# musaru/Fall_Multimodal

Measured on AMD Instinct MI355X. Metric: clips/sec (fwd+bwd) 3-stream Fall3, B=256, 1/2/4/8 GPUs; top-1 acc parity, higher is better.
Workload: dtype bf16x3; 1 GPU; fall3_3stream_coco_mmpose_V18_S6_B256_per_gpu; global_batch=256, seq_len=30, parallelism=dp1, joints=18, imu_axes=6, classes=11, hip_graph=False, ranks=1

## Files before the change

fall_multimodal_amd/_lib.py:

```python
from __future__ import annotations

import ctypes
import os

import torch

HERE = os.path.dirname(os.path.abspath(__file__))
LIB_PATH = os.environ.get("F3_LIB") or os.path.join(HERE, "libfall3.so")

EXPORTS = (
    "f3_net_create", "f3_net_destroy", "f3_net_num_entries", "f3_net_entry", "f3_net_param_count",
    "f3_net_buffer_count", "f3_net_counter_count", "f3_net_workspace_bytes", "f3_net_forward",
    "f3_net_loss", "f3_net_backward", "f3_rmsprop_step", "f3_conv_forward", "f3_status_string",
    "f3_net_debug_tensor", "f3_conv_backward_data", "f3_conv_backward_weight", "f3_conv_wgrad_packed", "f3_split_x3cat",
    "f3_conv_forward_x3cat", "f3_conv_backward_data_x3cat", "f3_conv_backward_weight_x3cat", "f3_conv_step_x3cat", "f3_graph_mix_forward",
    "f3_graph_mix_backward", "f3_graph_mix_forward_ex", "f3_graph_mix_backward_ex", "f3_gcn_dgrad_mix_x3",
    "f3_gcn_fwd_mix_x3",
    "f3_net_backward_phase",
    "f3_net_grad_split", "f3_net_wait_phase1", "f3_net_backward_rmsprop", "f3_net_fused_rmsprop", "f3_net_precision", "f3_net_status",
    "f3_targcn_create", "f3_targcn_destroy", "f3_targcn_num_entries", "f3_targcn_entry", "f3_targcn_param_count",
    "f3_targcn_buffer_count", "f3_targcn_workspace_bytes", "f3_targcn_forward", "f3_targcn_backward", "f3_targcn_stage_times", "f3_targcn_status", "f3_net_sensor_times", "f3_soft_ce",
    "f3_sktr_create", "f3_sktr_destroy", "f3_sktr_num_entries", "f3_sktr_entry", "f3_sktr_param_count",
    "f3_sktr_buffer_count", "f3_sktr_counter_count", "f3_sktr_workspace_bytes", "f3_sktr_forward", "f3_sktr_backward",
    "f3_musa_create", "f3_musa_destroy", "f3_musa_num_entries", "f3_musa_entry", "f3_musa_param_count",
    "f3_musa_buffer_count", "f3_musa_counter_count", "f3_musa_workspace_bytes", "f3_musa_forward", "f3_musa_backward",
    "f3_musa_guards",
    "f3_dwconv_t_forward", "f3_pointwise_conv", "f3_rgb_scratch_floats", "f3_rgb_forward", "f3_rgb_backward",
    "f3_optim_scalars_bytes", "f3_optim_step", "f3_optim_step_ranges", "f3_net_backward_optim", "f3_net_entry_nograd",
    "f3_metrics_bytes", "f3_metrics_reset", "f3_metrics_update", "f3_segment_norms_scratch_bytes", "f3_segment_norms",
    "f3_soft_ce_ex", "f3_net_loss_ex", "f3_grad_accumulate",
    "f3_optim_hyper_bytes", "f3_optim_hyper_set", "f3_optim_step_hyper",
)

F3_OK, F3_EINVAL, F3_EBATCH, F3_EHIP, F3_ESTATE, F3_EDEVICE = 0, 1001, 1002, 1003, 1004, 1005
ENTRY_PARAM, ENTRY_BUFFER, ENTRY_COUNTER = 0, 1, 2
OPT_RMSPROP, OPT_SGD, OPT_ADAM, OPT_ADAMW = 0, 1, 2, 3
OPT_MAX_SKIP = 4
METRICS_MAXK, METRICS_MAXC = 8, 64


# ... 69 lines not shown
        "f3_metrics_update": (I, [P, P, P, P, P, I, I, ctypes.POINTER(I), I, P]),
        "f3_segment_norms_scratch_bytes": (I64, [I64, I]),
        "f3_segment_norms": (I, [P, P, P, I, P, P, I64, ctypes.c_double, P]),
        "f3_soft_ce_ex": (I, [P, P, P, I, I, F, P, P, P]),
        "f3_net_loss_ex": (I, [P, I, P, P, F, P, P, P]),
        "f3_grad_accumulate": (I, [P, P, I64, P, P]),
        "f3_conv_forward": (I, [P, P, P, P, P, I, I, I, I, I, I, I, I, I, P]),
        "f3_status_string": (ctypes.c_char_p, [I]),
        "f3_net_debug_tensor": (P, [P, I, P, I, I, ctypes.c_char_p]),
        "f3_conv_backward_data": (I, [P, P, P, P, I, I, I, I, I, I, I, I, I, P]),
        "f3_conv_backward_weight": (I, [P, P, P, P, I, I, I, I, I, I, I, I, I, P]),
        "f3_conv_wgrad_packed": (I, [P, P, P, ctypes.c_longlong, I, I, I, I, I, I, I, I, P]),
        "f3_split_x3cat": (I, [P, P, ctypes.c_int64, I, P]),
        "f3_conv_forward_x3cat": (I, [P, P, P, P, P, I, I, I, I, I, I, I, I, P]),
        "f3_conv_backward_data_x3cat": (I, [P, P, P, P, I, I, I, I, I, I, I, I, P]),
        "f3_conv_backward_weight_x3cat": (I, [P, P, P, P, I, I, I, I, I, I, I, I, P]),
        "f3_conv_step_x3cat": (I, [I, P, P, P, P, P, P, P, P, P, P, F, P, P, I, I, I, I, I, P]),
        "f3_graph_mix_forward": (I, [P, P, P, I, I, I, I, P]),
        "f3_graph_mix_backward": (I, [P, P, P, P, P, I, I, I, I, P]),
        "f3_graph_mix_forward_ex": (I, [P, P, P, I, I, I, I, I, P]),
        "f3_graph_mix_backward_ex": (I, [P, P, P, P, P, I, I, I, I, I, P]),
        "f3_gcn_dgrad_mix_x3": (I, [P, P, P, P, P, P, P, I, I, I, I, I, I, I, P]),
        "f3_gcn_fwd_mix_x3": (I, [P, P, P, P, P, P, P, P, P, I, I, I, I, I, P]),
        "f3_targcn_create": (I, [ctypes.POINTER(F3TargcnConfig), ctypes.POINTER(P)]),
        "f3_targcn_destroy": (None, [P]),
        "f3_targcn_num_entries": (I, [P]),
        "f3_targcn_entry": (I, [P, I, ctypes.POINTER(ctypes.c_char_p), ctypes.POINTER(I), ctypes.POINTER(I),
                                ctypes.POINTER(I64), ctypes.POINTER(I64)]),
        "f3_targcn_param_count": (I64, [P]),
        "f3_targcn_buffer_count": (I64, [P]),
        "f3_targcn_workspace_bytes": (I64, [P, I]),
        "f3_targcn_stage_times": (I, [P, I, P]),
        "f3_targcn_status": (I, [P, I]),
        "f3_net_sensor_times": (I, [P, I, P]),
        "f3_targcn_forward": (I, [P, I, P, P, P, P, P, P]),
        "f3_targcn_backward": (I, [P, I, P, P, P, P, P, P]),
        "f3_soft_ce": (I, [P, P, I, I, P, P, P]),
        "f3_sktr_create": (I, [ctypes.POINTER(F3SktrConfig), ctypes.POINTER(P)]),
        "f3_sktr_destroy": (None, [P]),
        "f3_sktr_num_entries": (I, [P]),
        "f3_sktr_entry": (I, [P, I, ctypes.POINTER(ctypes.c_char_p), ctypes.POINTER(I), ctypes.POINTER(I),
                              ctypes.POINTER(I64), ctypes.POINTER(I64)]),
        "f3_sktr_param_count": (I64, [P]),
        "f3_sktr_buffer_count": (I64, [P]),
        "f3_sktr_counter_count": (I64, [P]),
        "f3_sktr_workspace_bytes": (I64, [P, I]),
# ... 49 lines not shown
```

fall_multimodal_amd/csrc/kernel_entries.cpp:

```cpp
#include <hip/hip_runtime.h>

#include <cstring>

#include "common.h"
#include "kernels.h"
#include "layers.h"
#include "host_args.h"
#include "fall3.h"

using namespace f3;

extern "C" {

static const unsigned short* test_zero_page() {
  static void* z = nullptr;
  if (!z && hipMalloc(&z, 4096) == hipSuccess) (void)hipMemset(z, 0, 4096);
  return (const unsigned short*)z;
}
static float* test_scratch(size_t n) {
  static float* p = nullptr;
  static size_t cap = 0;
  if (n > cap) {
    if (p) (void)hipFree(p);
    p = nullptr;
// ... 326 lines not shown
}

int f3_gcn_fwd_mix_x3(const float* A_eff, const float* x, const float* w, void* wpack, const float* bias_v, void* z3,
                      float* g, double* st_sum, double* st_sq, int frames, int K, int V, int Cin, int C,
                      void* stream) {
  hipStream_t s = (hipStream_t)stream;
  if (!A_eff || !x || !wpack || !bias_v || !z3 || !g || !st_sum || !st_sq || frames < 0) return F3_EINVAL;
  if (!f3_gcn_fwd_mix_ok(K, V, Cin, C)) return F3_EINVAL;
  if (w) {
    PrepTable t;
    t.n = 0;
    add_job(t, PREP_PACK_CONV, C * K * Cin * x3mul(x3code()), static_cast<float*>(wpack), w, nullptr, nullptr, C,
            K * Cin, 1, x3code());
    F3_TRY(f3_prep(t, s));
  }
  GcnFwdMixArgs a;
  std::memset(&a, 0, sizeof(a));
  a.frames = frames; a.K = K; a.V = V; a.Cin = Cin; a.C = C; a.A = A_eff; a.x = x;
  a.z3 = static_cast<unsigned short*>(z3); a.w = static_cast<const unsigned short*>(wpack); a.bias = bias_v; a.g = g;
  a.st_sum = st_sum; a.st_sq = st_sq; a.zero = test_zero_page();
  return f3_gcn_fwd_mix(&a, s);
}

}
```

fall_multimodal_amd/csrc/layers.h:

```cpp
#pragma once
#include "common.h"

namespace f3 {

enum : int { PREP_MUL = 0, PREP_PACK_CONV, PREP_PACK_CONV_T, PREP_PACK_GCN, PREP_PACK_GCN_T, PREP_GCN_BIAS, PREP_COPY,
              PREP_UNPACK_CONV };

struct PrepJob {
  int type, n;
  float* dst;
  const float* s0;
  const float* s1;
  const float* s2;
  int d0, d1, d2;
  int bf16;
};

struct DataBnArgs {
  int N, T, V, C, motion;
  const float* skel;
  float* out;
  int act16;
  BnRef bn;
  double* st_sum;
// ... 96 lines not shown
  unsigned short* outb;
  const float* dout;
  const float* dout_nc;
  float* P1;
  float* P2;
  float* Q2;
  double* bnr_bsum;
  double* bnr_bsq;
  const double* bn2_bsum;
  const double* bn2_bsq;
  const float* e;
  float* dh;
  float* dres;
  unsigned short* dhb;
  unsigned short* dresb;
  int x3;
  float* dgamma2;
  float* dbeta2;
  float* part;
  float* dgammar;
  float* dbetar;
  float* dbpart;
  int no_colsum;
};

struct BnBwdArgs {
  int N, TV, C, V, chunks;
  int act16;
  BnRef bn;
  const double* bsum;
  const double* bsq;
  float* dgamma;
  float* dbeta;
  const float* dv;
  const float* g;
  float* dg;
  float* G;
  float* Gpart;
  unsigned short* dgb;
  int no_colsum;
  int x3;
};

struct BnReluArgs {
  int M, C;
  int g16;
// ... 68 lines not shown
int f3_databn_bwd(const f3::DataBnArgs* a, hipStream_t s);
int f3_mix_fwd(const f3::MixArgs* a, hipStream_t s);
int f3_mix_bwd(const f3::MixArgs* a, hipStream_t s);
int f3_mix_bwd_parts(const f3::MixArgs* a);
bool f3_gcn_dgrad_mix_ok(int K, int V, int Cin, int C);
int f3_gcn_dgrad_mix(const f3::GcnDgradMixArgs* a, hipStream_t s);
int f3_gcn_dgrad_mix_parts(const f3::GcnDgradMixArgs* a);
bool f3_gcn_fwd_mix_ok(int K, int V, int Cin, int C);
int f3_gcn_fwd_mix(const f3::GcnFwdMixArgs* a, hipStream_t s);
bool f3_mix_lds_ok(int K, int V, int Cin);
bool f3_mix_x3_ok(int K, int V, int Cin);
int f3_split_x3(const float* x, unsigned short* out, long long rows, int C, hipStream_t s);
int f3_gcn_bias_bwd(const f3::GcnBiasBwdArgs* a, hipStream_t s);
bool f3_gcn0_ok(int K, int V, int Ci, int C);
int f3_gcn0_fwd(const f3::Gcn0Args* a, hipStream_t s);
int f3_gcn0_bwd(const f3::Gcn0Args* a, hipStream_t s);
int f3_gcn0_bwd_parts(const f3::Gcn0Args* a);
int f3_databn_bwd2(const f3::DataBnArgs* a, hipStream_t s);
int f3_block_out(f3::BlockArgs a, hipStream_t s);
int f3_block_bwd_reduce(f3::BlockArgs a, hipStream_t s);
int f3_block_bwd_apply(f3::BlockArgs a, hipStream_t s);
int f3_bn_bwd_apply(f3::BnBwdArgs a, hipStream_t s);
int f3_bn_bwd_parts(int N, int TV, int V);
int f3_block_chunks(int TV);
int f3_bnrelu_bf16(const f3::BnReluArgs* a, hipStream_t s);
constexpr int kColsumJobs = 10;
struct ColsumJob {
  const float* part;
  float* out;
  long long ld;
  int rows, cols;
};
int f3_colsum_multi(const ColsumJob* jobs, int n, hipStream_t s);
int f3_colsum(const float* part, int rows, int cols, float* out, hipStream_t s);
int f3_colsum_ld(const float* part, int rows, long long ld, int cols, float* out, hipStream_t s);
int f3_ca_fwd(const f3::CaArgs* a, hipStream_t s);
int f3_ca_bwd(const f3::CaArgs* a, hipStream_t s);
int f3_ca_bwd_weights(const f3::CaArgs* a, hipStream_t s, ColsumJob* defer = nullptr, int* ndefer = nullptr);
bool f3_ca_x_ok(int N, int C, int TV);
int f3_bn_running(const f3::BnRunTable& t, hipStream_t s);
```

fall_multimodal_amd/csrc/layers.hip:

```cpp
#include "common.h"
#include "layers.h"

#include <algorithm>
#include <cstring>
#include <type_traits>

namespace f3 {

typedef __bf16 bf16x4 __attribute__((ext_vector_type(4)));
typedef __bf16 bf16x8 __attribute__((ext_vector_type(8)));

F3_DEV void prep_x3n(const PrepJob& j, int e) {
  const bool gcn = j.type == PREP_PACK_GCN || j.type == PREP_PACK_GCN_T;
  const bool tr = j.type == PREP_PACK_CONV_T || j.type == PREP_PACK_GCN_T;
  const int J = j.d0, I = j.d1, KT = gcn ? 1 : j.d2;
  const int inner = gcn ? (tr ? J : j.d2 * I) : (tr ? J : I);
  const int row = e / (KT * inner), r = e - row * KT * inner, dt = r / inner, c = r - dt * inner;
  float val;
  if (gcn) {
    const int kc = tr ? row : c, cc = tr ? c : row, k = kc / I, ci = kc - k * I;
    val = j.s0[((size_t)k * J + cc) * I + ci];
  } else {
    val = tr ? j.s0[((size_t)c * I + row) * KT + dt] : j.s0[((size_t)row * I + c) * KT + dt];
  }
// ... 953 lines not shown
}

F3_DEV void chunk_rows(int TV, int chunks, int& r0, int& r1) {
  const int n = blockIdx.y, ch = blockIdx.x;
  const int per = (TV + chunks - 1) / chunks;
  r0 = n * TV + ch * per;
  r1 = min(n * TV + TV, r0 + per);
}

F3_DEV f32x4 quad_reduce(f32x4 v, float* lds, int C4) {
  const int tid = threadIdx.x;
  __syncthreads();
  reinterpret_cast<f32x4*>(lds)[tid] = v;
  __syncthreads();
  f32x4 r = {0.f, 0.f, 0.f, 0.f};
  if (tid < C4) {
    for (int i = tid; i < 256; i += C4) r += reinterpret_cast<f32x4*>(lds)[i];
  }
  return r;
}

constexpr int kRowU = 4;

template <bool A16, int RES>
__global__ __launch_bounds__(256) void block_out_kernel(BlockArgs a) {
  __shared__ __attribute__((aligned(16))) float lds[1024];
  const int C = a.C, C4 = C / 4, RP = 256 / C4, tid = threadIdx.x;
  int r0, r1;
  chunk_rows(a.TV, a.chunks, r0, r1);
  const int n = blockIdx.y, cq = tid % C4, c0 = cq * 4;
  const int mb0 = r0 + tid / C4;
  f32x4 h[kRowU], res[kRowU];
  size_t off[kRowU];
#define F3_BO_LOADS(MB)                                                  \
  _Pragma("unroll") for (int u = 0; u < kRowU; ++u) {                    \
    off[u] = (size_t)min((MB) + u * RP, r1 - 1) * C + c0;                \
    h[u] = ld_act4<A16>(a.h, off[u]);                                    \
    if (RES == RES_CONV) res[u] = ld_act4<A16>(a.r, off[u]);             \
    else if (RES == RES_ID) res[u] = ld_act4<A16>(a.x, off[u]);          \
    else res[u] = f32x4{0.f, 0.f, 0.f, 0.f};                             \
  }
  F3_BO_LOADS(mb0)
  float sc2[4], sh2[4], scr[4], shr[4], mu[4], rs[4];
  bn_coeff4(a.bn2, c0, sc2, sh2, mu, rs);
  if (RES == RES_CONV) bn_coeff4(a.bnr, c0, scr, shr, mu, rs);
  const f32x4 av = *reinterpret_cast<const f32x4*>(a.att + (size_t)n * C + c0);
  f32x4 pool = {0.f, 0.f, 0.f, 0.f};
  for (int mb = mb0; mb < r1; mb += kRowU * RP) {
    if (mb != mb0) F3_BO_LOADS(mb)
#pragma unroll
    for (int u = 0; u < kRowU; ++u) {
      f32x4 o;
#pragma unroll
      for (int e = 0; e < 4; ++e) {
        float rv = res[u][e];
        if (RES == RES_CONV) rv = rv * scr[e] + shr[e];
        o[e] = fmaxf((h[u][e] * sc2[e] + sh2[e]) * av[e] + rv, 0.f);
      }
      st_act4<A16>(a.out, off[u], o);
      if (a.outb) {
        bf16x4 ob, lb;
#pragma unroll
        for (int e = 0; e < 4; ++e) {
          ob[e] = (__bf16)o[e];
          lb[e] = (__bf16)(o[e] - (float)ob[e]);
        }
        if (a.x3) {
          __bf16* row = reinterpret_cast<__bf16*>(a.outb) + 2 * (off[u] - c0) + c0;
          *reinterpret_cast<bf16x4*>(row) = ob;
          *reinterpret_cast<bf16x4*>(row + C) = lb;
        } else {
          *reinterpret_cast<bf16x4*>(reinterpret_cast<__bf16*>(a.outb) + off[u]) = ob;
        }
      }
      if (mb + u * RP < r1) pool += o;
    }
  }
#undef F3_BO_LOADS
  if (a.pool) {
    f32x4 r = quad_reduce(pool, lds, C4);
    if (tid < C4) {
      if (a.part) {
        *reinterpret_cast<f32x4*>(a.part + ((size_t)blockIdx.x * a.N + n) * C + tid * 4) = r * a.inv_tv;
      } else {
#pragma unroll
        for (int e = 0; e < 4; ++e) atomic_add_f(a.pool + (size_t)n * C + tid * 4 + e, r[e] * a.inv_tv);
      }
    }
  }
}

template <bool A16, int RES, bool DNC>
__global__ __launch_bounds__(256) void block_bwd_reduce_kernel(BlockArgs a) {
  __shared__ __attribute__((aligned(16))) float lds[1024];
  const int C = a.C, C4 = C / 4, RP = 256 / C4, tid = threadIdx.x;
  int r0, r1;
  chunk_rows(a.TV, a.chunks, r0, r1);
  const int n = blockIdx.y, cq = tid % C4, c0 = cq * 4;
  const int mb0 = r0 + tid / C4;
  f32x4 o[kRowU], d[kRowU], h[kRowU], rr[kRowU];
#define F3_BR_LOADS(MB)                                                          \
  _Pragma("unroll") for (int u = 0; u < kRowU; ++u) {                            \
    const size_t off = (size_t)min((MB) + u * RP, r1 - 1) * C + c0;              \
    o[u] = ld_act4<A16>(a.out, off);                                             \
    if (!DNC) d[u] = *reinterpret_cast<const f32x4*>(a.dout + off);              \
    h[u] = ld_act4<A16>(a.h, off);                                               \
    if (RES == RES_CONV) rr[u] = ld_act4<A16>(a.r, off);                         \
  }
  F3_BR_LOADS(mb0)
  float mu2[4], rs2[4], mur[4], rsr[4], sc[4], sh[4];
  bn_coeff4(a.bn2, c0, sc, sh, mu2, rs2);
  if (RES == RES_CONV) bn_coeff4(a.bnr, c0, sc, sh, mur, rsr);
  f32x4 p1 = {0, 0, 0, 0}, p2 = {0, 0, 0, 0}, q2 = {0, 0, 0, 0};
  f32x4 dbc = {0, 0, 0, 0};
  if (DNC) dbc = *reinterpret_cast<const f32x4*>(a.dout_nc + (size_t)n * C + c0) * a.inv_tv;
  for (int mb = mb0; mb < r1; mb += kRowU * RP) {
    if (mb != mb0) F3_BR_LOADS(mb)
#pragma unroll
    for (int u = 0; u < kRowU; ++u) {
      const float w = mb + u * RP < r1 ? 1.f : 0.f;
#pragma unroll
      for (int e = 0; e < 4; ++e) {
        const float dz = o[u][e] > 0.f ? (DNC ? dbc[e] : d[u][e]) * w : 0.f;
        p1[e] += dz;
        p2[e] += dz * ((h[u][e] - mu2[e]) * rs2[e]);
        if (RES == RES_CONV) q2[e] += dz * ((rr[u][e] - mur[e]) * rsr[e]);
      }
    }
  }
#undef F3_BR_LOADS
  const size_t pblk = (size_t)a.N * C, prow = (size_t)blockIdx.x * 3 * pblk + (size_t)n * C + tid * 4;
  f32x4 s1 = quad_reduce(p1, lds, C4);
  if (tid < C4) {
    if (a.part) {
      *reinterpret_cast<f32x4*>(a.part + prow) = s1;
    } else {
#pragma unroll
      for (int e = 0; e < 4; ++e) atomic_add_f(a.P1 + (size_t)n * C + tid * 4 + e, s1[e]);
    }
  }
  f32x4 s2 = quad_reduce(p2, lds, C4);
  if (tid < C4) {
    if (a.part) {
      *reinterpret_cast<f32x4*>(a.part + pblk + prow) = s2;
    } else {
#pragma unroll
      for (int e = 0; e < 4; ++e) atomic_add_f(a.P2 + (size_t)n * C + tid * 4 + e, s2[e]);
    }
  }
  if (RES == RES_CONV) {
    f32x4 t2 = quad_reduce(q2, lds, C4);
    if (tid < C4) {
      if (a.part) {
        *reinterpret_cast<f32x4*>(a.part + 2 * pblk + prow) = t2;
      } else {
#pragma unroll
        for (int e = 0; e < 4; ++e) atomic_add_f(a.Q2 + (size_t)n * C + tid * 4 + e, t2[e]);
      }
    }
  }
}

template <bool A16, int RES, bool DNC>
__global__ __launch_bounds__(256) void block_bwd_apply_kernel(BlockArgs a) {
  const int C = a.C, C4 = C / 4, RP = 256 / C4, tid = threadIdx.x;
  const float invM = 1.f / (float)a.bn2.count;
  if (blockIdx.x == 0 && blockIdx.y == 0) {
    for (int c = tid; c < C; c += 256) {
      a.dgamma2[c] += (float)a.bn2_bsq[c];
      a.dbeta2[c] += (float)a.bn2_bsum[c];
      if (RES == RES_CONV) {
        a.dgammar[c] += (float)a.bnr_bsq[c];
        a.dbetar[c] += (float)a.bnr_bsum[c];
      }
    }
  }
  int r0, r1;
  chunk_rows(a.TV, a.chunks, r0, r1);
  const int n = blockIdx.y, cq = tid % C4, c0 = cq * 4;
  const int mb0 = r0 + tid / C4;
  f32x4 o[kRowU], d[kRowU], h[kRowU], rr[kRowU];
  size_t off[kRowU];
#define F3_BA_LOADS(MB)                                                          \
  _Pragma("unroll") for (int u = 0; u < kRowU; ++u) {                            \
    off[u] = (size_t)min((MB) + u * RP, r1 - 1) * C + c0;                        \
    o[u] = ld_act4<A16>(a.out, off[u]);                                          \
    if (!DNC) d[u] = *reinterpret_cast<const f32x4*>(a.dout + off[u]);           \
    h[u] = ld_act4<A16>(a.h, off[u]);                                            \
    if (RES == RES_CONV) rr[u] = ld_act4<A16>(a.r, off[u]);                      \
  }
  F3_BA_LOADS(mb0)
  float mu2[4], k2[4], m1[4], m2[4], rs2[4], mur[4], kr[4], n1[4], n2[4], rsr[4], sc[4], sh[4];
  double bs1[4], bs2[4], rs1[4], rsq[4];
#pragma unroll
  for (int e = 0; e < 4; ++e) {
    bs1[e] = a.bn2_bsum[c0 + e];
    bs2[e] = a.bn2_bsq[c0 + e];
    if (RES == RES_CONV) {
      rs1[e] = a.bnr_bsum[c0 + e];
      rsq[e] = a.bnr_bsq[c0 + e];
    }
  }
  bn_coeff4(a.bn2, c0, sc, sh, mu2, rs2);
  if (RES == RES_CONV) bn_coeff4(a.bnr, c0, sc, sh, mur, rsr);
#pragma unroll
  for (int e = 0; e < 4; ++e) {
    const int c = c0 + e;
    k2[e] = a.bn2.gamma[c] * rs2[e];
    m1[e] = (float)bs1[e] * invM;
    m2[e] = (float)bs2[e] * invM;
    if (RES == RES_CONV) {
      kr[e] = a.bnr.gamma[c] * rsr[e];
      n1[e] = (float)rs1[e] * invM;
      n2[e] = (float)rsq[e] * invM;
    }
  }
  const f32x4 av = *reinterpret_cast<const f32x4*>(a.att + (size_t)n * C + c0);
  const f32x4 ev = *reinterpret_cast<const f32x4*>(a.e + (size_t)n * C + c0);
  f32x4 dbc = {0, 0, 0, 0};
  if (DNC) dbc = *reinterpret_cast<const f32x4*>(a.dout_nc + (size_t)n * C + c0) * a.inv_tv;
  f32x4 sdh = {0, 0, 0, 0}, sdr = {0, 0, 0, 0};
  for (int mb = mb0; mb < r1; mb += kRowU * RP) {
    if (mb != mb0) F3_BA_LOADS(mb)
#pragma unroll
    for (int u = 0; u < kRowU; ++u) {
      f32x4 dh, dr;
#pragma unroll
      for (int e = 0; e < 4; ++e) {
        const float dz = o[u][e] > 0.f ? (DNC ? dbc[e] : d[u][e]) : 0.f;
        const float xh = (h[u][e] - mu2[e]) * rs2[e];
        dh[e] = k2[e] * (dz * av[e] + ev[e] - m1[e] - xh * m2[e]);
        if (RES == RES_CONV) {
          const float xr = (rr[u][e] - mur[e]) * rsr[e];
          dr[e] = kr[e] * (dz - n1[e] - xr * n2[e]);
        } else {
          dr[e] = dz;
        }
      }
      if (mb + u * RP < r1) {
        sdh += dh;
        if (RES == RES_CONV) sdr += dr;
      }
      if (a.dhb) {
        bf16x4 hb, lb;
#pragma unroll
        for (int e = 0; e < 4; ++e) {
          hb[e] = (__bf16)dh[e];
          lb[e] = (__bf16)(dh[e] - (float)hb[e]);
        }
        if (a.x3) {
          __bf16* row = reinterpret_cast<__bf16*>(a.dhb) + 2 * (off[u] - c0) + c0;
          *reinterpret_cast<bf16x4*>(row) = hb;
// ... 1142 lines not shown
  if (mix_lds_ok(*a)) {
    if (!a->part) return F3_EINVAL;
    const int r = a->Cin == 64 ? mix_bwd_cin<64>(a, s) : a->Cin == 128 ? mix_bwd_cin<128>(a, s) : mix_bwd_cin<256>(a, s);
    if (r >= 0) return r;
  }
  if (a->dzb) return F3_EINVAL;
  F3_BIG_LDS(mix_bwd_kernel);
  if (a->K * a->V * a->V > 1024 || mix_lds(*a, true) > 160 * 1024) return F3_EINVAL;
  const int grid = min(a->frames, 1024);
  hipLaunchKernelGGL(mix_bwd_kernel, dim3(grid), dim3(256), mix_lds(*a, true), s, *a);
  F3_LAUNCH_CHECK();
  return F3_OK;
}

int f3_gcn_bias_bwd(const GcnBiasBwdArgs* a, hipStream_t s) {
  if (a->K * a->V * a->V > 3072 || a->K * a->V > 1024) return F3_EINVAL;
  hipLaunchKernelGGL(gcn_bias_bwd_kernel, dim3((a->K * a->C + 255) / 256 + a->K * a->V), dim3(256), 0, s, *a);
  F3_LAUNCH_CHECK();
  return F3_OK;
}

static int chunks_for(int TV) { return max(1, (TV + 95) / 96); }
int f3_block_chunks(int TV) { return chunks_for(TV); }

template <bool A16, int RES, bool DNC>
static void launch_block_bwd1(const BlockArgs& a, bool reduce, hipStream_t s) {
  const dim3 grid(a.chunks, a.N);
  if (reduce) hipLaunchKernelGGL((block_bwd_reduce_kernel<A16, RES, DNC>), grid, dim3(256), 0, s, a);
  else hipLaunchKernelGGL((block_bwd_apply_kernel<A16, RES, DNC>), grid, dim3(256), 0, s, a);
}
template <bool A16, int RES>
static void launch_block_bwd2(const BlockArgs& a, bool reduce, hipStream_t s) {
  if (a.dout_nc) launch_block_bwd1<A16, RES, true>(a, reduce, s);
  else launch_block_bwd1<A16, RES, false>(a, reduce, s);
}
template <bool REDUCE>
static void launch_block_bwd(const BlockArgs& a, hipStream_t s) {
  if (a.act16) {
    if (a.res_kind == RES_CONV) launch_block_bwd2<true, RES_CONV>(a, REDUCE, s);
    else if (a.res_kind == RES_ID) launch_block_bwd2<true, RES_ID>(a, REDUCE, s);
    else launch_block_bwd2<true, RES_NONE>(a, REDUCE, s);
  } else {
    if (a.res_kind == RES_CONV) launch_block_bwd2<false, RES_CONV>(a, REDUCE, s);
    else if (a.res_kind == RES_ID) launch_block_bwd2<false, RES_ID>(a, REDUCE, s);
    else launch_block_bwd2<false, RES_NONE>(a, REDUCE, s);
  }
}

int f3_block_out(BlockArgs a, hipStream_t s) {
  if (a.C % 4 || a.C > 256 || 256 % (a.C / 4)) return F3_EINVAL;
  a.chunks = chunks_for(a.TV);
  if (!a.pool) a.part = nullptr;
// ... 211 lines not shown
```

fall_multimodal_amd/csrc/net.cpp:

```cpp
#include <hip/hip_runtime.h>

#include <algorithm>
#include <cstdio>
#include <cstdlib>
#include <cstring>
#include <string>
#include <vector>

#include "common.h"
#include "status_ring.h"
#include "kernels.h"
#include "layers.h"
#include "sensor.h"
#include "host_args.h"
#include "fall3.h"

using namespace f3;

namespace {

struct Entry {
  std::string name;
  int kind;
  std::vector<int64_t> shape;
// ... 48 lines not shown
struct LstmIdx {
  int wih[2], whh[2], bih[2], bhh[2];
  BnIdx bn;
  int ca_w1, ca_b1, ca_w2, ca_b2, fc_w, fc_b;
  int S, Cs;
};

struct CnnIdx {
  int w1, b1, w2, b2, fcw, fcb;
  BnIdx bn1, bn2;
};

const int kChan[7][4] = {{-1, 64, 1, RES_NONE}, {64, 64, 1, RES_ID},    {64, 64, 1, RES_ID},
                         {64, 128, 2, RES_CONV}, {128, 128, 1, RES_ID}, {128, 256, 2, RES_CONV},
                         {256, 256, 1, RES_ID}};

inline bool gcn_dgrad_fused() {
  static const bool on = !getenv("F3_GCN_DGRAD_FUSED") || atoi(getenv("F3_GCN_DGRAD_FUSED")) != 0;
  return on;
}

inline bool gcn_fwd_fused() {
  static const bool on = !getenv("F3_GCN_FWD_FUSED") || atoi(getenv("F3_GCN_FWD_FUSED")) != 0;
  return on;
}

LayerFmt layer_fmt(int precision, int K, int V, int Ci, int C, int res, bool next_res_conv) {
  const bool hb = precision == F3_PRECISION_BF16, x3 = precision == F3_PRECISION_BF16X3;
  LayerFmt f;
  const bool first = (hb || x3) && f3_gcn0_ok(K, V, Ci, C);
  f.gcat = x3 && f3_mix_x3_ok(K, V, Ci);
  f.dzb = hb && f3_mix_lds_ok(K, V, Ci);
  const bool fwd_fused = f.gcat && Ci == 64 && K * Ci == 192 && V <= 18 && (C == 64 || C == 128) && gcn_fwd_fused() &&
                         f3_gcn_fwd_mix_ok(K, V, Ci, C);
  const bool bwd_fused = f.gcat && Ci == 64 && gcn_dgrad_fused() && f3_gcn_dgrad_mix_ok(K, V, Ci, C);
  f.fwd = first ? GCN_FIRST : fwd_fused ? GCN_FUSED : GCN_PAIR;
  f.bwd = first ? GCN_FIRST : bwd_fused ? GCN_FUSED : GCN_PAIR;
  f.gop = hb ? OP_BF16 : f.gcat ? OP_HILO : x3 ? OP_F32X3 : OP_F32;
  f.top = hb ? OP_BF16 : x3 ? OP_HILO : OP_F32;
  const int wc = hb ? 1 : x3 ? 2 : 0;
  f.conv_code = x3 ? x3code() : wc;
  f.gcn_code = f.gcat ? x3code() : (x3 && first ? 0 : wc);
  f.z_w = 4;
  f.dg_w = 4;
  f.dres_w = res == RES_CONV ? 4 : 0;
  f.u_w = x3 ? 4 : hb ? 2 : 0;
// ... 166 lines not shown
  T* take(size_t n) {
    off = (off + 255) & ~(size_t)255;
    T* p = base ? reinterpret_cast<T*>(base + off) : nullptr;
    off += n * sizeof(T);
    return p;
  }
};

struct BnWs {
  double *fsum = nullptr, *fsq = nullptr, *bsum = nullptr, *bsq = nullptr;
};

struct LayerWs {
  const float* x = nullptr;
  float *z, *g, *h, *r = nullptr, *out, *q1, *hid, *att, *gap;
  float *gw, *gwT, *tw, *twT, *rw = nullptr, *rwT = nullptr, *aeff, *beff;
  BnWs bn1, bn2, bnr, bnca;
  float *P1, *P2, *Q2, *G, *dAeff, *dq2, *dbn, *dq1, *e;
  unsigned short *u = nullptr, *outb = nullptr;
  const unsigned short* xb = nullptr;
  float *dh = nullptr, *dg = nullptr, *dres = nullptr;
  float *gpart = nullptr, *mixpart = nullptr;
  float* dbpart = nullptr;
};

struct StreamWs {
  float *x0, *pool, *A;
  BnWs dbn;
  LayerWs L[7];
  float *dv, *dZ, *dx[2], *dpool;
  float* slab;
  float* detm;
  float* dets;
};

struct Ws {
  StreamWs st[2];
  float *y1, *p1, *y2, *p2, *dy1, *dp1, *dy2, *dp2;
  BnWs cbn1, cbn2, sbn;
  float* cpart = nullptr;
  int *csyncf = nullptr, *csyncb = nullptr;
  float *seq, *gates, *cell, *hmean, *ybn, *a1, *satt, *sout, *sdy, *sdpre2, *sdpre1, *dhmean;
  float* lwpart;
  float *out, *dlogits, *ds;
  float *skel, *sensor;
  char *zf0, *zf1, *zb0, *zb1;
// ... 35 lines not shown
    X.out = A.take<float>(Mo * C);
    X.q1 = A.take<float>((size_t)N * C / 4);
    X.hid = A.take<float>((size_t)N * C / 4);
    X.att = A.take<float>((size_t)N * C);
    X.gw = reinterpret_cast<float*>(A.take<unsigned short>((size_t)C * K * Ci * 2));
    X.gwT = reinterpret_cast<float*>(A.take<unsigned short>((size_t)C * K * Ci * 2));
    X.tw = reinterpret_cast<float*>(A.take<unsigned short>((size_t)C * 9 * C * 2));
    X.twT = reinterpret_cast<float*>(A.take<unsigned short>((size_t)C * 9 * C * 2));
    if (L.res == RES_CONV) {
      X.rw = reinterpret_cast<float*>(A.take<unsigned short>((size_t)C * Ci * 2));
      X.rwT = reinterpret_cast<float*>(A.take<unsigned short>((size_t)C * Ci * 2));
    }
    X.aeff = A.take<float>((size_t)K * V * V);
    X.beff = A.take<float>((size_t)V * C);
    X.dq2 = A.take<float>((size_t)N * C);
    X.dbn = A.take<float>((size_t)N * C / 4);
    X.dq1 = A.take<float>((size_t)N * C / 4);
    X.e = A.take<float>((size_t)N * C);
    X.dh = reinterpret_cast<float*>(A.take<unsigned short>(Mo * C * 2));
    X.dg = reinterpret_cast<float*>(A.take<char>(Mi * C * F.dg_w));
    X.gpart = A.take<float>((size_t)f3_bn_bwd_parts(N, L.T_in * V, V) * V * C);
    if (x3) X.dbpart = A.take<float>((size_t)f3_block_chunks(L.T_out * V) * N * 2 * C);
    X.mixpart = A.take<float>((size_t)kMixParts * K * V * V);
    if (F.dres_w) X.dres = reinterpret_cast<float*>(A.take<char>(Mo * C * F.dres_w));
    xin = X.out;
    xinb = hb ? reinterpret_cast<const unsigned short*>(X.out) : nullptr;
    if (F.outb_w) xinb = X.outb = reinterpret_cast<unsigned short*>(A.take<char>(Mo * C * F.outb_w));
    maxMC = std::max(maxMC, std::max(Mi * C, Mi * Ci));
    maxMC = std::max(maxMC, Mo * C);
    maxZ = std::max(maxZ, Mi * K * Ci);
  }

  W.dv = A.take<float>(maxMC);
  W.slab = A.take<float>(kWgradSlabFloats * (x3 ? 4 : 1));

  W.dZ = A.take<float>(maxZ);
  W.dx[0] = A.take<float>(maxMC);
  W.dx[1] = A.take<float>(maxMC);
  W.dpool = A.take<float>((size_t)N * 256);
  {
    size_t m = (size_t)((S.T * V + 95) / 96) * N * 256;
    size_t d = 0;
    for (int l = 0; l < 7; ++l) {
      const LayerIdx& L = S.L[l];
      const size_t ch = (size_t)(L.T_out * V + 95) / 96;
      m = std::max(m, 3 * ch * N * L.cout);
// ... 277 lines not shown
    set_in(ta, X.u, C, F.top);
    ta.zero = w.zero;
    F3_TRY(f3_conv_gemm(&ta, 0, EPI_BIAS | EPI_STATS | EPI_GAP, s));
  } else {
    set_in(ta, X.g, C, OP_F32);
    ta.pro_bn = bn1;
    F3_TRY(f3_conv_gemm(&ta, 1, EPI_BIAS | EPI_STATS | EPI_GAP, s));
  }
  CaArgs ca;
  std::memset(&ca, 0, sizeof(ca));
  ca.N = N; ca.C = C; ca.inv_tv = 1.f / (float)(To * V); ca.bn2 = bn2;
  ca.bnca = q.ref(L.bnca, X.bnca, (float)N, eval);
  ca.W1 = q.p(L.ca_w1); ca.b1 = q.p(L.ca_b1); ca.W2 = q.p(L.ca_w2); ca.b2 = q.p(L.ca_b2);
  ca.gapsum = X.gap; ca.q1 = X.q1; ca.hid = X.hid; ca.att = X.att; ca.ca_sum = X.bnca.fsum; ca.ca_sq = X.bnca.fsq;
  F3_TRY(f3_ca_fwd(&ca, s));
  BlockArgs ba;
  std::memset(&ba, 0, sizeof(ba));
  ba.N = N; ba.TV = To * V; ba.C = C; ba.res_kind = L.res; ba.inv_tv = 1.f / (float)(To * V);
  ba.bn2 = bn2; ba.bnr = bnr; ba.h = X.h; ba.r = X.r; ba.x = X.x; ba.att = X.att; ba.out = X.out;
  ba.pool = l == 6 ? W.pool : nullptr;
  ba.part = W.detm;
  ba.act16 = hb;
  if (F.outb_w) { ba.outb = X.outb; ba.x3 = 1; }
  F3_TRY(f3_block_out(ba, s));
  if (train) {
    add_bnrun(run, q, L.bn1, X.bn1.fsum, X.bn1.fsq, Mi);
    add_bnrun(run, q, L.bn2, X.bn2.fsum, X.bn2.fsq, Mo);
    if (L.res == RES_CONV) add_bnrun(run, q, L.bnr, X.bnr.fsum, X.bnr.fsq, Mo);
    add_bnrun(run, q, L.bnca, X.bnca.fsum, X.bnca.fsq, N);
  }
  return F3_OK;
}

RmsRanges layer_ranges(const Net& n, const LayerIdx& L) {
  RmsRanges r;
  r.n = 2;
  const Entry &a = n.entries[L.gcn_w], &b = n.entries[L.ca_b2], &e = n.entries[L.edge];
  r.lo[0] = a.offset;
  r.len[0] = b.offset + (b.numel + 3) / 4 * 4 - a.offset;
  r.lo[1] = e.offset;
  r.len[1] = (e.numel + 3) / 4 * 4;
  return r;
}

bool debug_stop(int si, int l) {
  static const char* e = getenv("F3_DEBUG_BWD_STOP");
// ... 92 lines not shown
  Ws& w = *c.w;
  StreamWs& W = w.st[c.si];
  const LayerIdx& L = net.st[c.si].L[c.l];
  const LayerFmt& F = L.fmt;
  LayerWs& X = W.L[c.l];
  const int K = net.K, V = net.V, N = c.N, l = c.l;
  const int hb = is_bf16(net), x3 = is_x3(net), wq = hb || x3;
  const int C = c.C, Ci = c.Ci, Ti = c.Ti, To = c.To, Mi = c.Mi;
  float* const dx = c.dx;
  BlockArgs ba;
  std::memset(&ba, 0, sizeof(ba));
  ba.N = N; ba.TV = To * V; ba.C = C; ba.res_kind = L.res; ba.inv_tv = 1.f / (float)(To * V);
  ba.bn2 = c.bn2; ba.bnr = c.bnr; ba.h = X.h; ba.r = X.r; ba.x = X.x; ba.att = X.att; ba.out = X.out;
  ba.dout = c.dout; ba.dout_nc = l == 6 ? W.dpool : nullptr; ba.act16 = hb;
  ba.P1 = X.P1; ba.P2 = X.P2; ba.Q2 = X.Q2; ba.bnr_bsum = X.bnr.bsum; ba.bnr_bsq = X.bnr.bsq;
  ba.bn2_bsum = X.bn2.bsum; ba.bn2_bsq = X.bn2.bsq; ba.e = X.e; ba.dh = X.dh;
  ba.dres = L.res == RES_CONV ? X.dres : (L.res == RES_ID ? dx : nullptr);
  ba.dhb = bfa(X.dh, F.top != OP_F32);
  ba.x3 = x3;
  ba.dresb = L.res == RES_CONV ? bfa(X.dres, F.top != OP_F32) : nullptr;
  ba.dgamma2 = q.g(L.bn2.w); ba.dbeta2 = q.g(L.bn2.b);
  if (L.res == RES_CONV) { ba.dgammar = q.g(L.bnr.w); ba.dbetar = q.g(L.bnr.b); }
  ba.part = W.detm;
  ba.no_colsum = c.ca_sums;
  F3_TRY(f3_block_bwd_reduce(ba, s));
  ba.no_colsum = 0;
  ba.dbpart = x3 ? X.dbpart : nullptr;
  F3_TRY(f3_ca_bwd(&c.ca, s));
  F3_TRY(f3_block_bwd_apply(ba, s));
  ConvGemmArgs td;
  std::memset(&td, 0, sizeof(td));
  td.g = geom(Mi, C, C, 9, L.stride, 4, 1, Ti, To, V, C, C);
  set_in(td, X.dh, C, F.top);
  td.zero = w.zero;
  td.w = X.twT; td.wb = bf(X.twT, wq); td.out = W.dv; td.aux = X.g; td.ldaux = C; td.epi_bn = c.bn1;
  td.outb = bfa(W.dv, hb); td.auxb = hb ? reinterpret_cast<const unsigned short*>(X.g) : nullptr;
  td.st_sum = X.bn1.bsum; td.st_sq = X.bn1.bsq;
  F3_TRY(f3_conv_gemm(&td, 0, EPI_RELUMASK, s));
  if (debug_stop(c.si, l)) return F3_OK;
  BnBwdArgs bb;
  std::memset(&bb, 0, sizeof(bb));
  bb.N = N; bb.TV = Ti * V; bb.C = C; bb.V = V; bb.bn = c.bn1; bb.bsum = X.bn1.bsum; bb.bsq = X.bn1.bsq;
  bb.dgamma = q.g(L.bn1.w); bb.dbeta = q.g(L.bn1.b); bb.dv = W.dv; bb.g = X.g; bb.dg = X.dg; bb.G = X.G;
  bb.Gpart = X.gpart; bb.dgb = bfa(X.dg, hb || F.gcat); bb.act16 = hb; bb.no_colsum = c.split;
  bb.x3 = F.gcat;
  F3_TRY(f3_bn_bwd_apply(bb, s));
// ... 704 lines not shown
int f3_net_wait_phase1(f3_net* net, void* stream) {
  if (!net) return F3_EINVAL;
  return wait_phase1(*net, (hipStream_t)stream);
}

int f3_rmsprop_step(float* params, float* square_avg, const float* grads, int64_t n, float lr, float alpha,
                    float eps, float grad_scale, void* stream) {
  if (!params || !square_avg || !grads) return F3_EINVAL;
  return f3_rmsprop(params, square_avg, grads, n, lr, alpha, eps, grad_scale, (hipStream_t)stream);
}

void* f3_net_debug_tensor(f3_net* net, int batch, void* workspace, int stream, int layer, const char* what) {
  if (!net || stream < 0 || stream >= net->nstreams || layer < 0 || layer > 6) return nullptr;
  Ws w = plan(*net, batch, (char*)workspace);
  StreamWs& W = w.st[stream];
  LayerWs& X = W.L[layer];
  const std::string k(what);
  if (k == "x") return (void*)X.x;
  if (k == "z") return X.z;
  if (k == "g") return X.g;
  if (k == "h") return X.h;
  if (k == "r") return X.r;
  if (k == "out") return X.out;
  if (k == "att") return X.att;
  if (k == "dh") return X.dh;
  if (k == "u") return X.u;
  if (k == "dv") return W.dv;
  if (k == "dg") return X.dg;
  if (k == "dZ") return W.dZ;
  if (k == "dres") return X.dres;
  if (k == "dx0") return W.dx[0];
  if (k == "dx1") return W.dx[1];
  if (k == "bn1_fsum") return X.bn1.fsum;
  if (k == "bn1_fsq") return X.bn1.fsq;
  if (k == "bn1_bsum") return X.bn1.bsum;
  if (k == "bn1_bsq") return X.bn1.bsq;
  if (k == "twT") return X.twT;
  if (k == "P1") return X.P1;
  if (k == "P2") return X.P2;
  if (k == "e") return X.e;
  if (k == "gap") return X.gap;
  if (k == "q1") return X.q1;
  if (k == "hid") return X.hid;
  if (k == "dq1") return X.dq1;
  if (k == "dq2") return X.dq2;
  if (k == "dbn") return X.dbn;
// ... 25 lines not shown
```

include/fall3.h:

```cpp
#ifndef FALL3_H
#define FALL3_H
#include <stdint.h>

#ifdef __cplusplus
extern "C" {
#endif

#define F3_OK 0
#define F3_EINVAL 1001
#define F3_EBATCH 1002
#define F3_EHIP 1003
#define F3_ESTATE 1004
#define F3_EDEVICE 1005

enum { F3_MODEL_TWO_STGCAN_BILSTM = 0, F3_MODEL_TWO_STGCAN = 1, F3_MODEL_STGCN = 2, F3_MODEL_BILSTM = 3 };
enum { F3_SENSOR_NONE = 0, F3_SENSOR_BILSTM = 1, F3_SENSOR_CNN_BILSTM = 2 };
enum { F3_NAMING_PACKAGE = 0, F3_NAMING_NOTEBOOK = 1 };
enum { F3_PRECISION_FP32 = 0,
       F3_PRECISION_BF16 = 1,
       F3_PRECISION_BF16_FP32IN = 2,
       F3_PRECISION_BF16X3 = 4  };
enum { F3_ENTRY_PARAM = 0, F3_ENTRY_BUFFER = 1, F3_ENTRY_COUNTER = 2 };

typedef struct f3_config {
// ... 126 lines not shown
                      double* st_sq, int N, int T_in, int T_out, int V, int Cin, int Cout, int stride, int transposed,
                      int epi, void* stream);

long long f3_rgb_scratch_floats(int B, int T);
int f3_rgb_forward(const void* frames, const void* wpack, const float* bias, float* feat, int B, int T, void* stream);
int f3_rgb_backward(const void* frames, const void* wpack, const float* bias, const float* dfeat, float* dw, float* db,
                    float* scratch, long long scratch_floats, int B, int T, void* stream);

int f3_graph_mix_forward(const float* A_eff, const float* x, float* z, int frames, int K, int V, int Cin,
                         void* stream);
int f3_graph_mix_backward(const float* A_eff, const float* x, const float* dz, float* dx, float* dA, int frames, int K,
                          int V, int Cin, void* stream);
enum { F3_MIX_X_BF16 = 1, F3_MIX_Z_BF16 = 2, F3_MIX_X3 = 4, F3_MIX_Z3 = 8 };
int f3_graph_mix_forward_ex(const float* A_eff, const void* x, void* z, int frames, int K, int V, int Cin, int flags,
                            void* stream);
int f3_graph_mix_backward_ex(const float* A_eff, const void* x, const void* dz, float* dx, float* dA, int frames, int K,
                             int V, int Cin, int flags, void* stream);
int f3_gcn_dgrad_mix_x3(const void* dg3, const float* w, void* wpack, const float* A_eff, const float* x, float* dx,
                        float* dA, int frames, int K, int V, int Cin, int C, int accumulate, int max_workgroups,
                        void* stream);
int f3_gcn_fwd_mix_x3(const float* A_eff, const float* x, const float* w, void* wpack, const float* bias_v, void* z3,
                      float* g, double* st_sum, double* st_sq, int frames, int K, int V, int Cin, int C,
                      void* stream);

const char* f3_status_string(int status);

typedef struct f3_targcn_config {
  int num_node;
  int num_class;
  int precision;
} f3_targcn_config;

typedef struct f3_targcn f3_targcn;

int f3_targcn_create(const f3_targcn_config* cfg, f3_targcn** out);
void f3_targcn_destroy(f3_targcn* net);
int f3_targcn_num_entries(const f3_targcn* net);
int f3_targcn_entry(const f3_targcn* net, int i, const char** name, int* kind, int* ndim, int64_t* shape8,
                    int64_t* offset);
int64_t f3_targcn_param_count(const f3_targcn* net);
int64_t f3_targcn_buffer_count(const f3_targcn* net);
int64_t f3_targcn_workspace_bytes(const f3_targcn* net, int batch);
int f3_targcn_forward(f3_targcn* net, int batch, const float* params, const float* buffers, const float* source,
                      float* out, void* workspace, void* stream);
int f3_targcn_backward(f3_targcn* net, int batch, const float* params, const float* buffers, const float* dout,
                       float* grads, void* workspace, void* stream);
// ... 62 lines not shown
```

Before: 33420 clips/s.

## Store ReLU sign bitmask in block forward and reuse it in backward

The block output kernel now packs a 16-bit mask per thread per row-trip recording which outputs are positive after ReLU, written to a new per-layer signs buffer. The backward reduce and apply kernels take a new SG template path that reads this mask instead of reloading the full output activation tensor, so each backward kernel reads much less from memory. It costs an extra small write in forward and a small workspace allocation per layer, and it adds a test entry point. The path is on by default and can be turned off with an environment variable.

```diff
diff --git a/fall_multimodal_amd/_lib.py b/fall_multimodal_amd/_lib.py
--- a/fall_multimodal_amd/_lib.py
+++ b/fall_multimodal_amd/_lib.py
@@ -15,7 +15,7 @@
     "f3_net_debug_tensor", "f3_conv_backward_data", "f3_conv_backward_weight", "f3_conv_wgrad_packed", "f3_split_x3cat",
     "f3_conv_forward_x3cat", "f3_conv_backward_data_x3cat", "f3_conv_backward_weight_x3cat", "f3_conv_step_x3cat", "f3_graph_mix_forward",
     "f3_graph_mix_backward", "f3_graph_mix_forward_ex", "f3_graph_mix_backward_ex", "f3_gcn_dgrad_mix_x3",
-    "f3_gcn_fwd_mix_x3",
+    "f3_gcn_fwd_mix_x3", "f3_block_signs_case",
     "f3_net_backward_phase",
     "f3_net_grad_split", "f3_net_wait_phase1", "f3_net_backward_rmsprop", "f3_net_fused_rmsprop", "f3_net_precision", "f3_net_status",
     "f3_targcn_create", "f3_targcn_destroy", "f3_targcn_num_entries", "f3_targcn_entry", "f3_targcn_param_count",
@@ -131,6 +131,7 @@
         "f3_graph_mix_backward_ex": (I, [P, P, P, P, P, I, I, I, I, I, P]),
         "f3_gcn_dgrad_mix_x3": (I, [P, P, P, P, P, P, P, I, I, I, I, I, I, I, P]),
         "f3_gcn_fwd_mix_x3": (I, [P, P, P, P, P, P, P, P, P, I, I, I, I, I, P]),
+        "f3_block_signs_case": (I, [I] + [P] * 13 + [ctypes.c_longlong] + [P] * 5 + [I] * 6 + [P]),
         "f3_targcn_create": (I, [ctypes.POINTER(F3TargcnConfig), ctypes.POINTER(P)]),
         "f3_targcn_destroy": (None, [P]),
         "f3_targcn_num_entries": (I, [P]),
diff --git a/fall_multimodal_amd/csrc/kernel_entries.cpp b/fall_multimodal_amd/csrc/kernel_entries.cpp
--- a/fall_multimodal_amd/csrc/kernel_entries.cpp
+++ b/fall_multimodal_amd/csrc/kernel_entries.cpp
@@ -372,4 +372,49 @@
   return f3_gcn_fwd_mix(&a, s);
 }
 
-}
+int f3_block_signs_case(int phases, const void* h, const void* r, const void* x, const float* att, const float* e,
+                        const float* bn2, const float* bnr, const double* bn2_b, const double* bnr_b,
+                        const float* dout, const float* dout_nc, void* out, void* signs, long long sign_words,
+                        float* part, void* dh, void* dres, float* dbpart, float* dgb, int N, int TV, int C,
+                        int res_kind, int act16, int x3, void* stream) {
+  hipStream_t s = (hipStream_t)stream;
+  if (N <= 0 || TV <= 0 || C < 4 || C % 4 || C > 256 || 256 % (C / 4)) return F3_EINVAL;
+  if (res_kind < RES_NONE || res_kind > RES_CONV || (act16 && x3)) return F3_EINVAL;
+  if (!h || !att || !bn2 || !out || (res_kind == RES_CONV && (!r || !bnr)) || (res_kind == RES_ID && !x)) return F3_EINVAL;
+  if (signs && sign_words < f3_block_sign_words(N, TV, C)) return F3_EINVAL;
+  BlockArgs a;
+  std::memset(&a, 0, sizeof(a));
+  a.N = N; a.TV = TV; a.C = C; a.res_kind = res_kind; a.inv_tv = 1.f / (float)TV; a.act16 = act16;
+  a.bn2.gamma = bn2; a.bn2.beta = bn2 + C; a.bn2.rmean = bn2 + 2 * C; a.bn2.rvar = bn2 + 3 * C;
+  a.bn2.count = (float)N * (float)TV; a.bn2.eval = 1;
+  if (res_kind == RES_CONV) {
+    a.bnr = a.bn2;
+    a.bnr.gamma = bnr; a.bnr.beta = bnr + C; a.bnr.rmean = bnr + 2 * C; a.bnr.rvar = bnr + 3 * C;
+  }
+  a.h = static_cast<const float*>(h); a.r = static_cast<const float*>(r); a.x = static_cast<const float*>(x);
+  a.att = att; a.out = static_cast<float*>(out); a.signs = static_cast<unsigned short*>(signs);
+  if (phases & 1) F3_TRY(f3_block_out(a, s));
+  if (!(phases & 2)) return F3_OK;
+  if (!e || !bn2_b || !part || !dh || !dgb || (!dout && !dout_nc) || (res_kind == RES_CONV && !bnr_b) ||
+      (res_kind != RES_NONE && !dres))
+    return F3_EINVAL;
+  a.dout = dout_nc ? nullptr : dout; a.dout_nc = dout_nc; a.e = e;
+  a.bn2_bsum = bn2_b; a.bn2_bsq = bn2_b + C;
+  if (res_kind == RES_CONV) {
+    a.bnr_bsum = const_cast<double*>(bnr_b); a.bnr_bsq = const_cast<double*>(bnr_b) + C;
+  }
+  a.dgamma2 = dgb; a.dbeta2 = dgb + C; a.dgammar = dgb + 2 * C; a.dbetar = dgb + 3 * C;
+  a.part = part; a.no_colsum = 1;
+  a.dh = static_cast<float*>(dh);
+  a.dres = static_cast<float*>(dres);
+  const bool gemm_rows = act16 || x3;
+  a.dhb = gemm_rows ? static_cast<unsigned short*>(dh) : nullptr;
+  a.dresb = gemm_rows && res_kind == RES_CONV ? static_cast<unsigned short*>(dres) : nullptr;
+  a.x3 = x3;
+  F3_TRY(f3_block_bwd_reduce(a, s));
+  a.no_colsum = 0;
+  a.dbpart = dbpart;
+  return f3_block_bwd_apply(a, s);
+}
+
+}
diff --git a/fall_multimodal_amd/csrc/layers.h b/fall_multimodal_amd/csrc/layers.h
--- a/fall_multimodal_amd/csrc/layers.h
+++ b/fall_multimodal_amd/csrc/layers.h
@@ -142,6 +142,7 @@
   float* dbetar;
   float* dbpart;
   int no_colsum;
+  unsigned short* signs;
 };
 
 struct BnBwdArgs {
@@ -256,6 +257,7 @@
 int f3_block_bwd_apply(f3::BlockArgs a, hipStream_t s);
 int f3_bn_bwd_apply(f3::BnBwdArgs a, hipStream_t s);
 int f3_bn_bwd_parts(int N, int TV, int V);
+long long f3_block_sign_words(int N, int TV, int C);
 int f3_block_chunks(int TV);
 int f3_bnrelu_bf16(const f3::BnReluArgs* a, hipStream_t s);
 constexpr int kColsumJobs = 10;
diff --git a/fall_multimodal_amd/csrc/layers.hip b/fall_multimodal_amd/csrc/layers.hip
--- a/fall_multimodal_amd/csrc/layers.hip
+++ b/fall_multimodal_amd/csrc/layers.hip
@@ -999,6 +999,14 @@
 
 constexpr int kRowU = 4;
 
+__host__ __device__ inline int block_sign_trips(int TV, int chunks, int C) {
+  const int per = (TV + chunks - 1) / chunks, rows = kRowU * (256 / (C / 4));
+  return (per + rows - 1) / rows;
+}
+F3_DEV size_t block_sign_base(const BlockArgs& a) {
+  return ((size_t)blockIdx.y * a.chunks + blockIdx.x) * block_sign_trips(a.TV, a.chunks, a.C) * 256 + threadIdx.x;
+}
+
 template <bool A16, int RES>
 __global__ __launch_bounds__(256) void block_out_kernel(BlockArgs a) {
   __shared__ __attribute__((aligned(16))) float lds[1024];
@@ -1023,8 +1031,10 @@
   if (RES == RES_CONV) bn_coeff4(a.bnr, c0, scr, shr, mu, rs);
   const f32x4 av = *reinterpret_cast<const f32x4*>(a.att + (size_t)n * C + c0);
   f32x4 pool = {0.f, 0.f, 0.f, 0.f};
+  unsigned short* sgw = a.signs ? a.signs + block_sign_base(a) : nullptr;
   for (int mb = mb0; mb < r1; mb += kRowU * RP) {
     if (mb != mb0) F3_BO_LOADS(mb)
+    unsigned sg = 0;
 #pragma unroll
     for (int u = 0; u < kRowU; ++u) {
       f32x4 o;
@@ -1033,6 +1043,8 @@
         float rv = res[u][e];
         if (RES == RES_CONV) rv = rv * scr[e] + shr[e];
         o[e] = fmaxf((h[u][e] * sc2[e] + sh2[e]) * av[e] + rv, 0.f);
+        const float stored = A16 ? (float)(__bf16)o[e] : o[e];
+        sg |= (stored > 0.f ? 1u : 0u) << (4 * u + e);
       }
       st_act4<A16>(a.out, off[u], o);
       if (a.outb) {
@@ -1052,6 +1064,10 @@
       }
       if (mb + u * RP < r1) pool += o;
     }
+    if (sgw) {
+      *sgw = (unsigned short)sg;
+      sgw += 256;
+    }
   }
 #undef F3_BO_LOADS
   if (a.pool) {
@@ -1067,7 +1083,7 @@
   }
 }
 
-template <bool A16, int RES, bool DNC>
+template <bool A16, int RES, bool DNC, bool SG>
 __global__ __launch_bounds__(256) void block_bwd_reduce_kernel(BlockArgs a) {
   __shared__ __attribute__((aligned(16))) float lds[1024];
   const int C = a.C, C4 = C / 4, RP = 256 / C4, tid = threadIdx.x;
@@ -1076,13 +1092,21 @@
   const int n = blockIdx.y, cq = tid % C4, c0 = cq * 4;
   const int mb0 = r0 + tid / C4;
   f32x4 o[kRowU], d[kRowU], h[kRowU], rr[kRowU];
-#define F3_BR_LOADS(MB)                                                          \
-  _Pragma("unroll") for (int u = 0; u < kRowU; ++u) {                            \
-    const size_t off = (size_t)min((MB) + u * RP, r1 - 1) * C + c0;              \
-    o[u] = ld_act4<A16>(a.out, off);                                             \
-    if (!DNC) d[u] = *reinterpret_cast<const f32x4*>(a.dout + off);              \
-    h[u] = ld_act4<A16>(a.h, off);                                               \
-    if (RES == RES_CONV) rr[u] = ld_act4<A16>(a.r, off);                         \
+  unsigned sg = 0;
+  const unsigned short* sgw = SG ? a.signs + block_sign_base(a) : nullptr;
+#define F3_BR_LOADS(MB)                                                            \
+  {                                                                                \
+    if (SG) {                                                                      \
+      sg = *sgw;                                                                   \
+      sgw += 256;                                                                  \
+    }                                                                              \
+    _Pragma("unroll") for (int u = 0; u < kRowU; ++u) {                            \
+      const size_t off = (size_t)min((MB) + u * RP, r1 - 1) * C + c0;              \
+      if (!SG) o[u] = ld_act4<A16>(a.out, off);                                    \
+      if (!DNC) d[u] = *reinterpret_cast<const f32x4*>(a.dout + off);              \
+      h[u] = ld_act4<A16>(a.h, off);                                               \
+      if (RES == RES_CONV) rr[u] = ld_act4<A16>(a.r, off);                         \
+    }                                                                              \
   }
   F3_BR_LOADS(mb0)
   float mu2[4], rs2[4], mur[4], rsr[4], sc[4], sh[4];
@@ -1098,7 +1122,8 @@
       const float w = mb + u * RP < r1 ? 1.f : 0.f;
 #pragma unroll
       for (int e = 0; e < 4; ++e) {
-        const float dz = o[u][e] > 0.f ? (DNC ? dbc[e] : d[u][e]) * w : 0.f;
+        const bool pos = SG ? (sg >> (4 * u + e)) & 1u : o[u][e] > 0.f;
+        const float dz = pos ? (DNC ? dbc[e] : d[u][e]) * w : 0.f;
         p1[e] += dz;
         p2[e] += dz * ((h[u][e] - mu2[e]) * rs2[e]);
         if (RES == RES_CONV) q2[e] += dz * ((rr[u][e] - mur[e]) * rsr[e]);
@@ -1138,7 +1163,7 @@
   }
 }
 
-template <bool A16, int RES, bool DNC>
+template <bool A16, int RES, bool DNC, bool SG>
 __global__ __launch_bounds__(256) void block_bwd_apply_kernel(BlockArgs a) {
   const int C = a.C, C4 = C / 4, RP = 256 / C4, tid = threadIdx.x;
   const float invM = 1.f / (float)a.bn2.count;
@@ -1158,13 +1183,21 @@
   const int mb0 = r0 + tid / C4;
   f32x4 o[kRowU], d[kRowU], h[kRowU], rr[kRowU];
   size_t off[kRowU];
-#define F3_BA_LOADS(MB)                                                          \
-  _Pragma("unroll") for (int u = 0; u < kRowU; ++u) {                            \
-    off[u] = (size_t)min((MB) + u * RP, r1 - 1) * C + c0;                        \
-    o[u] = ld_act4<A16>(a.out, off[u]);                                          \
-    if (!DNC) d[u] = *reinterpret_cast<const f32x4*>(a.dout + off[u]);           \
-    h[u] = ld_act4<A16>(a.h, off[u]);                                            \
-    if (RES == RES_CONV) rr[u] = ld_act4<A16>(a.r, off[u]);                      \
+  unsigned sg = 0;
+  const unsigned short* sgw = SG ? a.signs + block_sign_base(a) : nullptr;
+#define F3_BA_LOADS(MB)                                                            \
+  {                                                                                \
+    if (SG) {                                                                      \
+      sg = *sgw;                                                                   \
+      sgw += 256;                                                                  \
+    }                                                                              \
+    _Pragma("unroll") for (int u = 0; u < kRowU; ++u) {                            \
+      off[u] = (size_t)min((MB) + u * RP, r1 - 1) * C + c0;                        \
+      if (!SG) o[u] = ld_act4<A16>(a.out, off[u]);                                 \
+      if (!DNC) d[u] = *reinterpret_cast<const f32x4*>(a.dout + off[u]);           \
+      h[u] = ld_act4<A16>(a.h, off[u]);                                            \
+      if (RES == RES_CONV) rr[u] = ld_act4<A16>(a.r, off[u]);                      \
+    }                                                                              \
   }
   F3_BA_LOADS(mb0)
   float mu2[4], k2[4], m1[4], m2[4], rs2[4], mur[4], kr[4], n1[4], n2[4], rsr[4], sc[4], sh[4];
@@ -1204,7 +1237,8 @@
       f32x4 dh, dr;
 #pragma unroll
       for (int e = 0; e < 4; ++e) {
-        const float dz = o[u][e] > 0.f ? (DNC ? dbc[e] : d[u][e]) : 0.f;
+        const bool pos = SG ? (sg >> (4 * u + e)) & 1u : o[u][e] > 0.f;
+        const float dz = pos ? (DNC ? dbc[e] : d[u][e]) : 0.f;
         const float xh = (h[u][e] - mu2[e]) * rs2[e];
         dh[e] = k2[e] * (dz * av[e] + ev[e] - m1[e] - xh * m2[e]);
         if (RES == RES_CONV) {
@@ -2393,12 +2427,21 @@
 
 static int chunks_for(int TV) { return max(1, (TV + 95) / 96); }
 int f3_block_chunks(int TV) { return chunks_for(TV); }
-
+long long f3_block_sign_words(int N, int TV, int C) {
+  const int chunks = chunks_for(TV);
+  return (long long)chunks * N * block_sign_trips(TV, chunks, C) * 256;
+}
+
+template <bool A16, int RES, bool DNC, bool SG>
+static void launch_block_bwd0(const BlockArgs& a, bool reduce, hipStream_t s) {
+  const dim3 grid(a.chunks, a.N);
+  if (reduce) hipLaunchKernelGGL((block_bwd_reduce_kernel<A16, RES, DNC, SG>), grid, dim3(256), 0, s, a);
+  else hipLaunchKernelGGL((block_bwd_apply_kernel<A16, RES, DNC, SG>), grid, dim3(256), 0, s, a);
+}
 template <bool A16, int RES, bool DNC>
 static void launch_block_bwd1(const BlockArgs& a, bool reduce, hipStream_t s) {
-  const dim3 grid(a.chunks, a.N);
-  if (reduce) hipLaunchKernelGGL((block_bwd_reduce_kernel<A16, RES, DNC>), grid, dim3(256), 0, s, a);
-  else hipLaunchKernelGGL((block_bwd_apply_kernel<A16, RES, DNC>), grid, dim3(256), 0, s, a);
+  if (a.signs) launch_block_bwd0<A16, RES, DNC, true>(a, reduce, s);
+  else launch_block_bwd0<A16, RES, DNC, false>(a, reduce, s);
 }
 template <bool A16, int RES>
 static void launch_block_bwd2(const BlockArgs& a, bool reduce, hipStream_t s) {
diff --git a/fall_multimodal_amd/csrc/net.cpp b/fall_multimodal_amd/csrc/net.cpp
--- a/fall_multimodal_amd/csrc/net.cpp
+++ b/fall_multimodal_amd/csrc/net.cpp
@@ -94,6 +94,11 @@
 
 inline bool gcn_fwd_fused() {
   static const bool on = !getenv("F3_GCN_FWD_FUSED") || atoi(getenv("F3_GCN_FWD_FUSED")) != 0;
+  return on;
+}
+
+inline bool block_signs() {
+  static const bool on = !getenv("F3_BLOCK_SIGNS") || atoi(getenv("F3_BLOCK_SIGNS")) != 0;
   return on;
 }
 
@@ -306,6 +311,7 @@
   float *dh = nullptr, *dg = nullptr, *dres = nullptr;
   float *gpart = nullptr, *mixpart = nullptr;
   float* dbpart = nullptr;
+  unsigned short* signs = nullptr;
 };
 
 struct StreamWs {
@@ -387,6 +393,7 @@
     X.gpart = A.take<float>((size_t)f3_bn_bwd_parts(N, L.T_in * V, V) * V * C);
     if (x3) X.dbpart = A.take<float>((size_t)f3_block_chunks(L.T_out * V) * N * 2 * C);
     X.mixpart = A.take<float>((size_t)kMixParts * K * V * V);
+    if (block_signs()) X.signs = A.take<unsigned short>((size_t)f3_block_sign_words(N, L.T_out * V, C));
     if (F.dres_w) X.dres = reinterpret_cast<float*>(A.take<char>(Mo * C * F.dres_w));
     xin = X.out;
     xinb = hb ? reinterpret_cast<const unsigned short*>(X.out) : nullptr;
@@ -710,6 +717,7 @@
   ba.part = W.detm;
   ba.act16 = hb;
   if (F.outb_w) { ba.outb = X.outb; ba.x3 = 1; }
+  ba.signs = train ? X.signs : nullptr;
   F3_TRY(f3_block_out(ba, s));
   if (train) {
     add_bnrun(run, q, L.bn1, X.bn1.fsum, X.bn1.fsq, Mi);
@@ -848,6 +856,7 @@
   ba.dgamma2 = q.g(L.bn2.w); ba.dbeta2 = q.g(L.bn2.b);
   if (L.res == RES_CONV) { ba.dgammar = q.g(L.bnr.w); ba.dbetar = q.g(L.bnr.b); }
   ba.part = W.detm;
+  ba.signs = X.signs;
   ba.no_colsum = c.ca_sums;
   F3_TRY(f3_block_bwd_reduce(ba, s));
   ba.no_colsum = 0;
@@ -1598,6 +1607,7 @@
   if (k == "h") return X.h;
   if (k == "r") return X.r;
   if (k == "out") return X.out;
+  if (k == "signs") return X.signs;
   if (k == "att") return X.att;
   if (k == "dh") return X.dh;
   if (k == "u") return X.u;
diff --git a/include/fall3.h b/include/fall3.h
--- a/include/fall3.h
+++ b/include/fall3.h
@@ -172,6 +172,11 @@
 int f3_gcn_fwd_mix_x3(const float* A_eff, const float* x, const float* w, void* wpack, const float* bias_v, void* z3,
                       float* g, double* st_sum, double* st_sq, int frames, int K, int V, int Cin, int C,
                       void* stream);
+int f3_block_signs_case(int phases, const void* h, const void* r, const void* x, const float* att, const float* e,
+                        const float* bn2, const float* bnr, const double* bn2_b, const double* bnr_b,
+                        const float* dout, const float* dout_nc, void* out, void* signs, long long sign_words,
+                        float* part, void* dh, void* dres, float* dbpart, float* dgb, int N, int TV, int C,
+                        int res_kind, int act16, int x3, void* stream);
 
 const char* f3_status_string(int status);
 
```

Result: faster. 33800 clips/s, median of 6 (+1.2%).
